# Distributed-Learning-Networking-Group/torchgpipe

Measured on AMD Instinct MI355X. Metric: U-Net(5,64) GPipe training throughput (samples/sec), higher is better.
Workload: dtype fp32; 1 GPU; model=U-Net(5,64), experiment=pipeline-1, global_batch=80, input=3x192x192, chunks=2, checkpoint=except_last, parallelism=pp1, transport=none, fused_cells=True, cell_streams=0, overlap_recompute=True, overlap_forward=True, graph_cells=False, hw_queues=4

## Files before the change

torchgpipe_amd/csrc/bindings.cpp:

```cpp
#include <algorithm>
#include <torch/extension.h>
#include <ATen/hip/HIPContext.h>
#include <ATen/hip/impl/HIPGuardImplMasqueradingAsCUDA.h>

#include <vector>

#include "aten_checks.h"
#include "kernels.h"

namespace tgpipe {
namespace {

hipStream_t stream_of(const at::Tensor& t) {
  return at::hip::getCurrentHIPStream(t.device().index()).stream();
}

const int64_t* rng_state(const c10::optional<at::Tensor>& rng, const at::Device& device) {
  if (!rng.has_value() || !rng->defined()) return nullptr;
  TORCH_CHECK(rng->is_cuda() && rng->device() == device && rng->scalar_type() == at::kLong &&
                  rng->is_contiguous() && rng->numel() == 2,
              "rng must be a contiguous int64 [2] (seed, offset) tensor on the op's device");
  return rng->data_ptr<int64_t>();
}

// ... 232 lines not shown
              "input too large for the F(4x4) kernel (needs < 1 GiB); use wino_conv");
  const float* bptr = nullptr;
  if (bias.has_value() && bias->defined()) {
    check_f32_gpu(*bias, "bias");
    TORCH_CHECK(bias->numel() == out_channels, "bias must have K elements");
    bptr = bias->data_ptr<float>();
  }
  c10::hip::HIPGuardMasqueradingAsCUDA guard(x.device());
  auto y = at::empty({n, out_channels, h, w}, x.options());
  if (y.numel() == 0) return y;
  TORCH_CHECK(variant == -1 || wino4_variant_known(static_cast<int>(variant)),
              "variant must be -1, 4-10, 12, 14-18, 20-22 or 24");
  const WinoPlan plan = wino4_plan(n, r, h, w, out_channels, static_cast<int>(variant),
                                   static_cast<int>(splits));
  at::Tensor ws;
  if (plan.workspace > 0) ws = at::empty({plan.workspace}, x.options());
  launch_wino4_conv(x.data_ptr<float>(), u.data_ptr<float>(), bptr, y.data_ptr<float>(),
                    plan.workspace > 0 ? ws.data_ptr<float>() : nullptr, n, r, h, w,
                    out_channels, plan, stream_of(x));
  return y;
}

at::Tensor wgrad_destination(const c10::optional<at::Tensor>& into, const at::Tensor& x,
                             int64_t k, int64_t c) {
  if (!into.has_value()) return at::empty({k, c, 3, 3}, x.options());
  const at::Tensor& d = *into;
  TORCH_CHECK(d.is_contiguous() && d.scalar_type() == at::kFloat && d.device() == x.device() &&
                  d.dim() == 4 && d.size(0) == k && d.size(1) == c && d.size(2) == 3 &&
                  d.size(3) == 3,
              "into must be a contiguous fp32 [K][C][3][3] tensor on x's device");
  return d;
}

at::Tensor wino_wgrad(const at::Tensor& x_in, const at::Tensor& dy_in, int64_t splits,
                      int64_t variant, const c10::optional<at::Tensor>& into) {
  auto x = x_in.contiguous();
  auto dy = dy_in.contiguous();
  check_f32_gpu(x, "x");
  check_f32_gpu(dy, "dy");
  TORCH_CHECK(x.dim() == 4 && dy.dim() == 4, "x and dy must be NCHW");
  const int64_t n = x.size(0), c = x.size(1), h = x.size(2), w = x.size(3), k = dy.size(1);
  TORCH_CHECK(dy.size(0) == n && dy.size(2) == h && dy.size(3) == w,
              "dy must be [N][K][H][W] of a 3x3/s1/p1 convolution of x");
  TORCH_CHECK(dy.device() == x.device(), "x and dy must share a device");
  TORCH_CHECK(c * h * w < (int64_t{1} << 31) && k * h * w < (int64_t{1} << 31),
              "plane too large for 32-bit channel offsets");
  c10::hip::HIPGuardMasqueradingAsCUDA guard(x.device());
  const bool accum = into.has_value();
  auto dw = wgrad_destination(into, x, k, c);
  if (n == 0 || h == 0 || w == 0) return accum ? dw : dw.zero_();
  TORCH_CHECK(variant == -1 || variant == 0 || variant == 2, "variant must be -1, 0 or 2");
  const int64_t tiles = n * ((h + 1) / 2) * ((w + 1) / 2);
  int v = variant >= 0 ? static_cast<int>(variant) : (k <= 32 ? 0 : 2);
  if (v == 2 && tiles >= (int64_t{1} << 24)) v = 0;
  const int64_t steps = (tiles + 7) / 8;
  const int s = static_cast<int>(std::min<int64_t>(
      splits > 0 ? splits : wino_wgrad_splits(n, c, k, h, w, v), steps));
  at::Tensor ws;
  if (s > 1) ws = at::empty({s * k * c * 9}, x.options());
  launch_wino_wgrad(x.data_ptr<float>(), dy.data_ptr<float>(), dw.data_ptr<float>(),
                    s > 1 ? ws.data_ptr<float>() : nullptr, n, c, k, h, w, s, v, accum,
                    stream_of(x));
  return dw;
}

at::Tensor wino4_wgrad(const at::Tensor& x_in, const at::Tensor& dy_in, int64_t splits,
                       int64_t variant, const c10::optional<at::Tensor>& into) {
  auto x = x_in.contiguous();
  auto dy = dy_in.contiguous();
  check_f32_gpu(x, "x");
  check_f32_gpu(dy, "dy");
  TORCH_CHECK(x.dim() == 4 && dy.dim() == 4, "x and dy must be NCHW");
  const int64_t n = x.size(0), c = x.size(1), h = x.size(2), w = x.size(3), k = dy.size(1);
  TORCH_CHECK(dy.size(0) == n && dy.size(2) == h && dy.size(3) == w,
              "dy must be [N][K][H][W] of a 3x3/s1/p1 convolution of x");
  TORCH_CHECK(dy.device() == x.device(), "x and dy must share a device");
  c10::hip::HIPGuardMasqueradingAsCUDA guard(x.device());
  const bool accum = into.has_value();
  auto dw = wgrad_destination(into, x, k, c);
  if (n == 0 || h == 0 || w == 0 || c == 0 || k == 0) return accum ? dw : dw.zero_();
  TORCH_CHECK(wino4_wgrad_supported(n, c, k, h, w),
              "input too large for the F(4x4) weight-gradient kernel (needs < 1 GiB); "
              "use wino_wgrad");
  TORCH_CHECK(variant >= 0 && variant <= 3,
              "variant must be 0 (fused), 1 (non-fused), 2 (split-bf16 batched GEMM) or 3 (fused, "
              "x rows through LDS)");
  const WinoPlan plan = wino4_wgrad_plan(n, c, k, h, w, static_cast<int>(variant),
                                         static_cast<int>(splits));
  at::Tensor ws;
  if (plan.workspace > 0) ws = at::empty({plan.workspace}, x.options());
  launch_wino4_wgrad(x.data_ptr<float>(), dy.data_ptr<float>(), dw.data_ptr<float>(),
                     plan.workspace > 0 ? ws.data_ptr<float>() : nullptr, n, c, k, h, w, plan,
                     accum, stream_of(x));
  return dw;
}

at::Tensor bg_weight(const at::Tensor& w, bool flip, int64_t kind,
                     const c10::optional<at::Tensor>& out, int64_t emu) {
  check_f32_gpu(w, "weight");
  TORCH_CHECK(w.dim() == 4 && w.size(2) == 3 && w.size(3) == 3, "weight must be [K][C][3][3]");
  auto wc = w.contiguous();
  const int64_t out_channels = flip ? w.size(1) : w.size(0);
  const int64_t red_channels = flip ? w.size(0) : w.size(1);
  c10::hip::HIPGuardMasqueradingAsCUDA guard(w.device());
  TORCH_CHECK(kind == 4 || kind == 2, "kind must be 4 (F(4x4)) or 2 (F(2x2))");
  auto a =
      transform_out(out, {bg_weight_numel(out_channels, red_channels, static_cast<int>(kind),
                                          static_cast<int>(emu))}, w);
  launch_bg_weight(wc.data_ptr<float>(), a.data_ptr<float>(), out_channels, red_channels, flip,
                   static_cast<int>(kind), stream_of(w), static_cast<int>(emu));
  return a;
}

at::Tensor bg_conv(const at::Tensor& x_in, const at::Tensor& a,
                   const c10::optional<at::Tensor>& bias, int64_t out_channels, int64_t bn,
                   int64_t splits, int64_t kind, int64_t waves, int64_t sub, int64_t emu,
                   const c10::optional<at::Tensor>& stats) {
  auto x = x_in.contiguous();
  check_f32_gpu(x, "x");
  check_f32_gpu(a, "a");
  TORCH_CHECK(x.dim() == 4, "x must be NCHW");
  const int64_t n = x.size(0), r = x.size(1), h = x.size(2), w = x.size(3);
  TORCH_CHECK(kind == 4 || kind == 2, "kind must be 4 (F(4x4)) or 2 (F(2x2))");
  TORCH_CHECK(a.dim() == 1 && a.numel() == bg_weight_numel(out_channels, r, static_cast<int>(kind),
                                                           static_cast<int>(emu)),
              "batched-GEMM transformed weight does not match the input/output channels");
  TORCH_CHECK(a.device() == x.device(), "a must live on the input's device");
  TORCH_CHECK(wino4_supported(n, r, h, w, out_channels),
              "input too large for the F(4x4) kernels (needs < 1 GiB)");
  const float* bptr = nullptr;
  if (bias.has_value() && bias->defined()) {
    check_f32_gpu(*bias, "bias");
    TORCH_CHECK(bias->numel() == out_channels, "bias must have K elements");
    bptr = bias->data_ptr<float>();
  }
  c10::hip::HIPGuardMasqueradingAsCUDA guard(x.device());
  auto y = at::empty({n, out_channels, h, w}, x.options());
  if (n == 0 || h == 0 || w == 0 || out_channels == 0) return y;
  const BgPlan plan = bg_plan(n, r, h, w, out_channels, static_cast<int>(bn),
                              static_cast<int>(splits), static_cast<int>(kind),
                              static_cast<int>(waves), static_cast<int>(sub),
                              static_cast<int>(emu));
  TORCH_CHECK(plan.ksteps * 16 * plan.np < (int64_t{1} << 31) &&
                  plan.mp * plan.np < (int64_t{1} << 31),
              "operands too large for the batched-GEMM kernels");
  float* pm = nullptr;
  int ipg = 0;
  if (stats.has_value() && stats->defined()) {
    check_f32_gpu(*stats, "stats");
    ipg = bg_stats_ipg(n, h, w, static_cast<int>(kind));
    const int64_t groups = (n + ipg - 1) / ipg;
    TORCH_CHECK(stats->device() == x.device() && stats->is_contiguous() &&
                    stats->numel() == 2 * groups * out_channels,
                "stats must be a contiguous [2][ceil(n / bg_stats_ipg)][K] float32 tensor");
    pm = stats->data_ptr<float>();
  }
  auto ws = at::empty({plan.workspace}, x.options());
  launch_bg_conv(x.data_ptr<float>(), a.data_ptr<float>(), bptr, y.data_ptr<float>(),
                 ws.data_ptr<float>(), n, r, h, w, out_channels, plan, stream_of(x), pm,
                 pm == nullptr ? nullptr : pm + stats->numel() / 2, ipg);
  return y;
}

int64_t bg_stats_images(int64_t n, int64_t h, int64_t w, int64_t kind) {
  return bg_stats_ipg(n, h, w, static_cast<int>(kind));
}

int64_t wino4_splits(int64_t n, int64_t c, int64_t k, int64_t h, int64_t w, int64_t variant) {
  if (variant == 0) return wino4_wgrad_plan(n, c, k, h, w, 0, 0).splits;
// ... 88 lines not shown
```

torchgpipe_amd/csrc/winograd_f4.hip:

```cpp
#include <hip/hip_runtime.h>
#include <stdint.h>

#include <algorithm>
#include <cstdlib>
#include <string>
#include <type_traits>

#include "kernels.h"

namespace tgpipe {
namespace {

typedef float floatx4 __attribute__((ext_vector_type(4)));
typedef float floatx2 __attribute__((ext_vector_type(2)));

constexpr int kP = 36;
constexpr int kC = 4;
constexpr int kOPad = 64;
constexpr int kT = 32;
constexpr int kVImg = kC * kT * kP;

template <int OG>
struct F4Cfg {
  static constexpr int kO = 16 * OG;
// ... 1979 lines not shown
  char* const vmine =
      vimg + (pt >> 4) * kEBlock + (((pc >> 3) * 16 + (pt & 15)) * 8 + (pc & 7)) * 2;
  const uint32_t chunk_bytes = static_cast<uint32_t>(kEC) * HW * 4;

  const int g = lane >> 4, row = lane & 15;
  const int a32 = wo * kEBlock + ((g & 1) * 16 + row) * 16;
  const int a16 = wo * kEBlock + 512 + ((g >> 1) * 16 + row) * 16 + (g & 1) * 8;
  const int b32 = wt * kEBlock + lane * 16;
  const int b16 = wt * kEBlock + ((g >> 1) * 16 + row) * 16 + (g & 1) * 8;

  const char* const ubase = reinterpret_cast<const char*>(u);
  const int64_t ochunk = static_cast<int64_t>(Op / 64);
  auto issue_slice = [&](int chunk, int pg, int slot) {
    const char* src = ubase + ((static_cast<int64_t>(chunk) * ochunk + ob) * kP + pg * kEPG) * 4 *
                                  kEBlock;
    char* dst = uring + slot * kEUSlice;
#pragma unroll
    for (int i = 0; i < 3; ++i) {
      const int piece = i * 8 + wave;
      __builtin_amdgcn_global_load_lds((glob_void_t*)(src + piece * 1024 + lane * 16),
                                       (lds_void_t*)(dst + piece * 1024), 16, 0, 0);
    }
  };

  if (c_begin < c_end) issue_slice(c_begin, 0, 0);
  for (int ck = c_begin; ck < c_end; ++ck) {
    f4_load_patch<kVec>(p, xr, ck * chunk_bytes);
    if (ck * kEC + pc >= R) {
#pragma unroll
      for (int b = 0; b < kP; ++b) p.d[b] = 0.f;
    }
    f4_transform(p);
#pragma unroll
    for (int b = 0; b < kP; ++b) {
      const __bf16 h = static_cast<__bf16>(p.d[b]);
      const __bf16 m = static_cast<__bf16>(p.d[b] - static_cast<float>(h));
      *reinterpret_cast<__bf16*>(vmine + b * 2 * kEBlock) = h;
      *reinterpret_cast<__bf16*>(vmine + b * 2 * kEBlock + 512) = m;
    }
    __syncthreads();
#pragma unroll
    for (int pg = 0; pg < kP / kEPG; ++pg) {
      const int slot = pg & 1;
      if (pg + 1 < kP / kEPG) {
        issue_slice(ck, pg + 1, slot ^ 1);
      } else if (ck + 1 < c_end) {
        issue_slice(ck + 1, 0, slot ^ 1);
      }
      const char* us = uring + slot * kEUSlice;
#pragma unroll
      for (int hq = 0; hq < kEPG; hq += 3) {
        bf16x8 fa[3], fb[3];
        shortx4 ga[3], gb[3];
#pragma unroll
        for (int q = 0; q < 3; ++q) {
          const int pos = pg * kEPG + hq + q;
          fa[q] = *reinterpret_cast<const bf16x8*>(us + (hq + q) * 4 * kEBlock + a32);
          fb[q] = *reinterpret_cast<const bf16x8*>(vimg + pos * 2 * kEBlock + b32);
          ga[q] = *reinterpret_cast<const shortx4*>(us + (hq + q) * 4 * kEBlock + a16);
          gb[q] = *reinterpret_cast<const shortx4*>(vimg + pos * 2 * kEBlock + b16);
        }
#pragma unroll
        for (int q = 0; q < 3; ++q) {
          const int pos = pg * kEPG + hq + q;
          acc[pos] = __builtin_amdgcn_mfma_f32_16x16x32_bf16(fa[q], fb[q], acc[pos], 0, 0, 0);
        }
#pragma unroll
        for (int q = 0; q < 3; ++q) {
          const int pos = pg * kEPG + hq + q;
          acc[pos] = __builtin_amdgcn_mfma_f32_16x16x16bf16_1k(ga[q], gb[q], acc[pos], 0, 0, 0);
        }
      }
      __builtin_amdgcn_sched_barrier(0);
      __syncthreads();
      __builtin_amdgcn_sched_barrier(0);
    }
  }

  const int tp = t0 + wt * 16 + (lane & 15);
  if (tp >= P) return;
  float* ydst = y + static_cast<int64_t>(z) * (P / tpi) * O * HW;
  f4_output_transform(acc, ydst, bias != nullptr && splits == 1 ? bias : nullptr, tp, tpi, TW,
                      H, W, O, o0 + wo * 16 + 4 * (lane >> 4));
}

__global__ __launch_bounds__(256) void bg_output_f4_kernel(
    const float* __restrict__ cbuf, const float* __restrict__ bias, float* __restrict__ y, int O,
    int Mp, int Np, int P, int tpi, int TW, int H, int W, int splits) {
  const int64_t idx = static_cast<int64_t>(blockIdx.x) * blockDim.x + threadIdx.x;
  if (idx >= static_cast<int64_t>(O) * P) return;
  const int t = static_cast<int>(idx % P);
  const int o = static_cast<int>(idx / P);
  const int64_t pos = static_cast<int64_t>(Mp) * Np;
  const float* src = cbuf + static_cast<int64_t>(o) * Np + t;
  float m[kP];
#pragma unroll
  for (int b = 0; b < kP; ++b) m[b] = src[b * pos];
  for (int z = 1; z < splits; ++z) {
    const float* sz = src + static_cast<int64_t>(z) * kP * pos;
#pragma unroll
    for (int b = 0; b < kP; ++b) m[b] += sz[b * pos];
  }
  float s[4][6];
#pragma unroll
  for (int jc = 0; jc < 6; ++jc) {
    const float a = m[6 + jc] + m[12 + jc], bq = m[6 + jc] - m[12 + jc];
    const float cc = m[18 + jc] + m[24 + jc], d = m[18 + jc] - m[24 + jc];
    s[0][jc] = m[jc] + a + cc;
    s[1][jc] = bq + 2.f * d;
    s[2][jc] = a + 4.f * cc;
    s[3][jc] = bq + 8.f * d + m[30 + jc];
  }
  const float bv = bias ? bias[o] : 0.f;
  const int n = t / tpi;
  const int rem = t - n * tpi;
  const int ty = rem / TW;
  const int py = 4 * ty, px = 4 * (rem - ty * TW);
  float* yp = y + (static_cast<int64_t>(n) * O + o) * H * W + static_cast<int64_t>(py) * W + px;
  const bool full = (W & 3) == 0 && py + 4 <= H;
#pragma unroll
  for (int k = 0; k < 4; ++k) {
    const float a = s[k][1] + s[k][2], bq = s[k][1] - s[k][2];
    const float cc = s[k][3] + s[k][4], d = s[k][3] - s[k][4];
    const floatx4 out{s[k][0] + a + cc + bv, bq + 2.f * d + bv, a + 4.f * cc + bv,
                      bq + 8.f * d + s[k][5] + bv};
    if (full) {
      *reinterpret_cast<floatx4*>(yp + k * W) = out;
    } else if (py + k < H) {
#pragma unroll
      for (int l = 0; l < 4; ++l)
        if (px + l < W) yp[k * W + l] = out[l];
    }
  }
}

constexpr int kP2 = 16;

__device__ __forceinline__ void f2_weight_tile(const float* __restrict__ w, int O, int R, int m,
                                               int r, bool flip, float (&v)[kP2]) {
  float g[3][3] = {};
  if (r < R && m < O) {
    const float* src = flip ? w + (static_cast<int64_t>(r) * O + m) * 9
                            : w + (static_cast<int64_t>(m) * R + r) * 9;
#pragma unroll
    for (int i = 0; i < 3; ++i)
#pragma unroll
      for (int jc = 0; jc < 3; ++jc) g[i][jc] = flip ? src[(2 - i) * 3 + (2 - jc)] : src[i * 3 + jc];
  }
  float t[4][3];
#pragma unroll
  for (int jc = 0; jc < 3; ++jc) {
    t[0][jc] = g[0][jc];
    t[1][jc] = 0.5f * (g[0][jc] + g[1][jc] + g[2][jc]);
    t[2][jc] = 0.5f * (g[0][jc] - g[1][jc] + g[2][jc]);
    t[3][jc] = g[2][jc];
  }
#pragma unroll
  for (int i = 0; i < 4; ++i) {
    v[i * 4 + 0] = t[i][0];
    v[i * 4 + 1] = 0.5f * (t[i][0] + t[i][1] + t[i][2]);
    v[i * 4 + 2] = 0.5f * (t[i][0] - t[i][1] + t[i][2]);
    v[i * 4 + 3] = t[i][2];
  }
}


// ... 752 lines not shown
  hipLaunchKernelGGL(plan.kind == 2 ? bg_output_f2_kernel : bg_output_f4_kernel,
                     dim3(static_cast<unsigned>((ot + 255) / 256)), dim3(256),
                     0, stream, cbuf, bias, y, static_cast<int>(out_channels),
                     static_cast<int>(plan.mp), static_cast<int>(plan.np), static_cast<int>(P),
                     static_cast<int>(th * tw), static_cast<int>(tw), static_cast<int>(h),
                     static_cast<int>(w), plan.splits);
}



namespace {
struct WgEmuPlan {
  int64_t ksteps, mp, np;
  int bn;
};

WgEmuPlan wg_emu_plan(int64_t n, int64_t c, int64_t k, int64_t h, int64_t w) {
  WgEmuPlan p;
  const int64_t P = n * ((h + 3) / 4) * ((w + 3) / 4);
  p.ksteps = (P + 15) / 16;
  p.bn = bg_pick_bn(c, 4, true);
  p.mp = bg_round(k, 128);
  p.np = bg_round(c, p.bn);
  return p;
}

int wg_emu_splits(const WgEmuPlan& p) {
  const int64_t tiles = (p.mp / 128) * (p.np / p.bn) * kP;
  int64_t s = 1;
  while (tiles * s < 1024 && p.ksteps / (s * 2) >= 8) s *= 2;
  return static_cast<int>(s);
}

int64_t wg_emu_workspace(const WgEmuPlan& p, int splits) {
  return bg_image_numel(kP, p.ksteps, p.mp + p.np, true) +
         static_cast<int64_t>(splits) * kP * p.mp * p.np;
}

void launch_wgrad_emu(const float* x, const float* dy, float* dw, float* ws, int64_t n,
                      int64_t c, int64_t k, int64_t h, int64_t w, int splits, bool accum,
                      hipStream_t stream) {
  const WgEmuPlan p = wg_emu_plan(n, c, k, h, w);
  const int64_t th = (h + 3) / 4, tw = (w + 3) / 4;
  const int64_t P = n * th * tw;
  float* am = ws;
  float* bv = am + bg_image_numel(kP, p.ksteps, p.mp, true);
  float* cb = bv + bg_image_numel(kP, p.ksteps, p.np, true);
  const bool vec = (w & 3) == 0;
  const int64_t mt = p.ksteps * 4 * p.mp, vt = p.ksteps * 4 * p.np;
  hipLaunchKernelGGL(vec ? wg_dy_emu_kernel<true> : wg_dy_emu_kernel<false>,
                     dim3(static_cast<unsigned>((mt + 255) / 256)), dim3(256), 0, stream, dy, am,
                     static_cast<int>(n), static_cast<int>(k), static_cast<int>(h),
                     static_cast<int>(w), static_cast<int>(th), static_cast<int>(tw),
                     static_cast<int>(p.mp), static_cast<int>(p.ksteps),
                     static_cast<uint32_t>(n * k * h * w * 4));
  hipLaunchKernelGGL(vec ? wg_x_emu_kernel<true> : wg_x_emu_kernel<false>,
                     dim3(static_cast<unsigned>((vt + 255) / 256)), dim3(256), 0, stream, x, bv,
                     static_cast<int>(c), static_cast<int>(h), static_cast<int>(w),
                     static_cast<int>(tw), static_cast<int>(th * tw), static_cast<int>(P),
                     static_cast<int>(p.np), static_cast<int>(p.ksteps),
                     static_cast<uint32_t>(n * c * h * w * 4));
  const int mtiles = static_cast<int>(p.mp / 128);
  const int ntiles = static_cast<int>(p.np / p.bn);
  const int64_t nwg = static_cast<int64_t>(mtiles) * ntiles * kP * splits;
  auto gemm = bg_emu_gemm(p.bn);
  hipLaunchKernelGGL(gemm, dim3(static_cast<unsigned>(nwg)), dim3(256), 0, stream, am, bv, cb,
                     static_cast<int>(p.mp), static_cast<int>(p.np), static_cast<int>(p.ksteps),
                     mtiles, ntiles, static_cast<int>(kP), splits);
  const int64_t ot = k * c;
  hipLaunchKernelGGL(wg_output_emu_kernel, dim3(static_cast<unsigned>((ot + 255) / 256)),
                     dim3(256), 0, stream, cb, dw, static_cast<int>(k), static_cast<int>(c),
                     static_cast<int>(p.mp), static_cast<int>(p.np), splits, accum);
}
}


bool wino4_wgrad_supported(int64_t n, int64_t c, int64_t k, int64_t h, int64_t w) {
  const int64_t lim = (int64_t{1} << 30) - 64;
  const int64_t tiles = n * ((h + 3) / 4) * ((w + 3) / 4);
  return n * c * h * w * 4 < lim && n * k * h * w * 4 < lim && n * c * h * w > 0 &&
         n * k * h * w > 0 && tiles + 64 < (int64_t{1} << 30);
}

WinoPlan wino4_wgrad_plan(int64_t n, int64_t c, int64_t k, int64_t h, int64_t w, int variant,
                          int splits) {
  WinoPlan plan;
  plan.variant = variant >= 1 && variant <= 3 ? variant : 0;
  if (plan.variant == 3 && ((w & 3) != 0 || w < 16)) plan.variant = 0;
  const int64_t tiles = n * ((h + 3) / 4) * ((w + 3) / 4);
  const int64_t cpad = (c + 31) / 32 * 32, kpad = (k + 63) / 64 * 64;
  const bool emu = plan.variant == 2;
  const WgEmuPlan p = wg_emu_plan(n, c, k, h, w);
  const int64_t steps = emu ? (tiles + 15) / 16 : (tiles + 3) / 4;
  int64_t s = splits;
  if (s <= 0 && emu) s = wg_emu_splits(p);
  if (s <= 0) {
    const double mb = static_cast<double>(cpad) * kpad * 9 * 4 / 1e6;
    s = split_k_by_cost((cpad / 32) * (kpad / 64), steps, 256, 2.5, 5.0, 0.8, mb, 512);
  }
  plan.splits = static_cast<int>(std::min(s, steps));
  plan.workspace = plan.splits > 1 ? plan.splits * k * c * 9 : 0;
  if (plan.variant == 1) plan.workspace += steps * 4 * (cpad + kpad) * kP;
  if (emu) plan.workspace = wg_emu_workspace(p, plan.splits);
  return plan;
}

void launch_wino4_wgrad(const float* x, const float* dy, float* dw, float* ws, int64_t n,
                        int64_t c, int64_t k, int64_t h, int64_t w, const WinoPlan& plan,
                        bool accum, hipStream_t stream) {
  const int splits = plan.splits;
  if (plan.variant == 2) {
    launch_wgrad_emu(x, dy, dw, ws, n, c, k, h, w, splits, accum, stream);
    return;
  }
  const int64_t th = (h + 3) / 4, tw = (w + 3) / 4;
  const int64_t P = n * th * tw;
  const int cblocks = static_cast<int>((c + 31) / 32);
  const int kblocks = static_cast<int>((k + 63) / 64);
  const int64_t nwg = static_cast<int64_t>(cblocks) * kblocks * splits;
  const uint32_t x_bytes = static_cast<uint32_t>(n * c * h * w * 4);
  const uint32_t dy_bytes = static_cast<uint32_t>(n * k * h * w * 4);
  float* partial = ws;
  if (plan.variant == 1) {
    const int64_t nsteps = (P + 3) / 4;
    const int64_t ppad = nsteps * 4;
    float* vx = ws;
    float* m = vx + ppad * cblocks * 32 * kP;
    partial = m + ppad * kblocks * 64 * kP;
    const int64_t vt = ppad * cblocks * 32, mt = ppad * kblocks * 64;
    hipLaunchKernelGGL(f4_wg_vx_kernel, dim3(static_cast<unsigned>((vt + 255) / 256)), dim3(256), 0,
                       stream, x, vx, static_cast<int>(n), static_cast<int>(c), static_cast<int>(h),
                       static_cast<int>(w), static_cast<int>(th), static_cast<int>(tw),
                       static_cast<int>(ppad), cblocks, vt, x_bytes);
    auto mk = (w & 3) == 0 ? f4_wg_mdy_kernel<true> : f4_wg_mdy_kernel<false>;
    hipLaunchKernelGGL(mk, dim3(static_cast<unsigned>((mt + 255) / 256)), dim3(256), 0, stream, dy,
                       m, static_cast<int>(n), static_cast<int>(k), static_cast<int>(h),
                       static_cast<int>(w), static_cast<int>(th), static_cast<int>(tw),
                       static_cast<int>(ppad), kblocks, mt, dy_bytes);
    hipLaunchKernelGGL(f4_wgrad_gemm_kernel<>, dim3(static_cast<unsigned>(nwg)), dim3(kWgThreads), 0,
                       stream, vx, m, splits > 1 ? partial : dw, static_cast<int>(c),
                       static_cast<int>(k), static_cast<int>(nsteps), cblocks, kblocks, splits,
                       accum && splits == 1);
  } else {
    auto kernel = (w & 3) == 0 ? f4_wgrad_kernel<true> : f4_wgrad_kernel<false>;
    if (plan.variant == 3) kernel = f4_wgrad_rows_kernel;
    hipLaunchKernelGGL(kernel, dim3(static_cast<unsigned>(nwg)), dim3(kWgThreads), 0,
                       stream, x, dy, splits > 1 ? partial : dw, static_cast<int>(n),
                       static_cast<int>(c), static_cast<int>(k), static_cast<int>(h),
                       static_cast<int>(w), static_cast<int>(th), static_cast<int>(tw),
                       static_cast<int>(P), cblocks, kblocks, splits, x_bytes, dy_bytes,
                       accum && splits == 1);
  }
  if (splits > 1) {
    launch_split_reduce(partial, nullptr, dw, k * c * 9, 9, static_cast<int>(k), splits, stream,
                        accum);
  }
}

}
```

torchgpipe_amd/ops/conv.py:

```python
import os
import threading
from typing import Any, Dict, List, Optional, Sequence, Tuple
import weakref

import torch
from torch import Tensor, nn
import torch.nn.functional as F

from torchgpipe_amd.ops import _ext, gradacc, precision
from torchgpipe_amd.ops.precision import autocast_lowp

__all__ = ['WinogradConv2d', 'winograd_conv2d', 'wino_eligible', 'new_step',
           'clear_winograd_caches', 'cache_bytes', 'refresh_step_caches', 'hold_cache',
           'size_cache_budget', 'conv_with_bn_stats']

_STEP = 0
_CACHE_BYTES: Dict[torch.device, int] = {}
_BUDGET: Optional[int] = None
_DEVICE_BUDGET: Dict[torch.device, int] = {}
_FRACTION = os.environ.get('TGPIPE_WINOGRAD_CACHE_FRACTION')
CACHE_PEAK_FRACTION: Optional[float] = float(_FRACTION) if _FRACTION else None
PRESPLIT_MB = max(0, int(os.environ.get('TGPIPE_CG_PRESPLIT_MB', '2048')))


# ... 315 lines not shown
        db = None
        if ctx.has_bias and ctx.needs_input_grad[2]:
            db = dy.sum((0, 2, 3))
        return dx, dw, db, None


class _WinogradConvStats(torch.autograd.Function):

    @staticmethod
    def forward(ctx, x: Tensor, weight: Tensor, cache: _TransformCache,
                kind: int) -> Tuple[Tensor, Tensor]:
        ops = _ext.require(x)
        x = x.contiguous()
        n, _, h, w = x.shape
        k = weight.shape[0]
        groups = -(-n // ops.bg_stats_images(n, h, w, kind))
        stats = torch.empty(2, groups, k, device=x.device, dtype=torch.float32)
        y = ops.bg_conv(x, cache.get(weight, False, bg=kind), None, k, 0, 0, kind,
                        stats=stats)
        ctx.save_for_backward(x, weight)
        ctx.cache = cache
        ctx.param = weight
        ctx.mark_non_differentiable(stats)
        ctx.set_materialize_grads(False)
        return y, stats

    @staticmethod
    def backward(ctx, dy: Optional[Tensor], _dstats: Optional[Tensor]):
        if dy is None:
            ctx.param = None
            return None, None, None, None
        x, weight = ctx.saved_tensors
        dx, dw = _conv_grads(x, weight, dy.contiguous(), ctx.cache, ctx.needs_input_grad[0],
                             ctx.needs_input_grad[1], ctx.param)
        ctx.param = None
        return dx, dw, None, None


BG_BN_STATS = os.environ.get('TGPIPE_BG_BN_STATS', '1') != '0'


def conv_with_bn_stats(module: nn.Conv2d, x: Tensor
                       ) -> Optional[Tuple[Tensor, Tensor, int]]:
    if not BG_BN_STATS or module.bias is not None:
        return None
    kind = _bg_kind(x, module.out_channels)
    if not kind:
        return None
    y, stats = _WinogradConvStats.apply(x, module.weight, module._wino, kind)
    n, _, h, w = x.shape
    return y, stats, _ext.require(x).bg_stats_images(n, h, w, kind)


def _conv_grads(x: Tensor, weight: Tensor, dy: Tensor, cache: _TransformCache, need_x: bool,
                need_w: bool, param: Optional[Tensor] = None
                ) -> Tuple[Optional[Tensor], Optional[Tensor]]:
    dx = dw = None
    if need_x:
        dx = _conv(dy, cache, weight, None, True)
    if need_w:
        ops = _ext.require(dy)
        f4, mfma = _wgrad_f4(x, dy, weight), _wgrad_on_mfma(x, weight)
        fuse, into = gradacc.target(param) if param is not None else (False, None)
        if f4:
            dw = ops.wino4_wgrad(x, dy, 0, _wgrad_f4_variant(x, weight), into)
        elif mfma:
            dw = ops.wino_wgrad(x, dy, 0, -1, into)
        else:
            dw = torch.ops.aten.convolution_backward(
                dy, x, weight, None, [1, 1], [1, 1], [1, 1], False, [0, 0], 1,
                [False, True, False])[1]
        if fuse:
            assert param is not None
            if into is None:
                gradacc.commit(param, dw)
            elif not (f4 or mfma):
                into.add_(dw)
            dw = None
    return dx, dw


WGRAD_EMU = os.environ.get('TGPIPE_WGRAD_EMU', '1') != '0'
WGRAD_EMU_MIN_TILES = 320


def _wgrad_f4_variant(x: Tensor, weight: Tensor) -> int:
    if min(weight.shape[0], weight.shape[1]) < 512:
        return 3 if x.shape[3] % 4 == 0 and x.shape[3] >= F4_ROWS_MIN_WIDTH else 0
    tiles = x.shape[0] * -(-x.shape[2] // 4) * -(-x.shape[3] // 4)
    return 2 if WGRAD_EMU and tiles >= WGRAD_EMU_MIN_TILES else 1


def _wgrad_f4(x: Tensor, dy: Tensor, weight: Tensor) -> bool:
    plane = min(x.shape[2], x.shape[3])
    wide = min(weight.shape[0], weight.shape[1]) >= F4_WIDE_CHANNELS
    return (F4_ENABLED and weight.shape[1] >= 16
            and (plane >= F4_MIN_PLANE or (plane >= F4_MIN_PLANE_WIDE and wide))
            and x.numel() * x.element_size() < F4_MAX_BYTES
            and dy.numel() * dy.element_size() < F4_MAX_BYTES)


def _wgrad_on_mfma(x: Tensor, weight: Tensor) -> bool:
    k, c = weight.shape[0], weight.shape[1]
    if k > 32:
        return c >= 16
    return c >= 64 and x.shape[2] * x.shape[3] >= 96 * 96


MIN_CHANNELS = 8


WINOGRAD_ENABLED = os.environ.get('TGPIPE_WINOGRAD', '1') != '0'

MAX_TRANSFORM_BYTES = int(float(os.environ.get('TGPIPE_WINOGRAD_MAX_TRANSFORM_MB', '2048'))
                          * (1 << 20))


WEIGHT_DOMINATED_RATIO = float(os.environ.get('TGPIPE_WINOGRAD_WEIGHT_RATIO', '256'))


def _transform_ratio(x: Tensor, weight: Tensor) -> float:
    positions = 16 if min(x.shape[2], x.shape[3]) < F4_MIN_PLANE else 36
    return weight.shape[0] * weight.shape[1] * positions / max(1, x.numel())


def wino_eligible(x: Tensor, weight: Tensor, stride: Sequence[int] = (1, 1),
                  padding: Sequence[int] = (1, 1), dilation: Sequence[int] = (1, 1),
                  groups: int = 1) -> bool:
    return (WINOGRAD_ENABLED and x.is_cuda and x.dim() == 4 and x.dtype == torch.float32
            and not autocast_lowp('cuda')
            and weight.shape[1] >= MIN_CHANNELS
            and weight.shape[0] * weight.shape[1] * 16 * 4 <= MAX_TRANSFORM_BYTES
            and weight.dtype == torch.float32 and tuple(weight.shape[2:]) == (3, 3)
            and tuple(stride) == (1, 1) and tuple(padding) == (1, 1)
            and tuple(dilation) == (1, 1) and groups == 1
            and _transform_ratio(x, weight) <= WEIGHT_DOMINATED_RATIO)


def winograd_conv2d(x: Tensor, weight: Tensor, bias: Optional[Tensor] = None,
                    cache: Optional[_TransformCache] = None) -> Tensor:
    if not wino_eligible(x, weight):
        return F.conv2d(x, weight, bias, padding=1)
    return _WinogradConv.apply(x, weight, bias, cache or _TransformCache())


class WinogradConv2d(nn.Conv2d):

    def __init__(self, *args, **kwargs) -> None:
        super().__init__(*args, **kwargs)
        self._wino = _TransformCache()

    def forward(self, input: Tensor) -> Tensor:
        if self.padding_mode == 'zeros' and wino_eligible(input, self.weight, self.stride,
                                                          self.padding, self.dilation,
                                                          self.groups):
            return _WinogradConv.apply(input, self.weight, self.bias, self._wino)
        from torchgpipe_amd.ops.convbn import gemm_conv2d, gemm_conv_eligible
        if WINOGRAD_ENABLED and self.weight.shape[1] < MIN_CHANNELS and \
                gemm_conv_eligible(input, self):
            return gemm_conv2d(input, self)
        return super().forward(input)

    def __getstate__(self):
        state = self.__dict__.copy()
        state['_wino'] = _TransformCache()
        return state
```

Before: 720.1 samples/sec.

## Add fused split-bf16 F(4x4) Winograd weight-gradient kernel for small-channel layers

Adds a new weight-gradient kernel variant (4) that transforms x and dy tiles in LDS, splits each value into three bf16 parts, and accumulates with bf16 MFMAs to emulate fp32 precision. It uses 32x32 channel blocks with two wave phases that each handle half of the 36 Winograd positions, then reduces the halves through LDS. The dispatcher routes specific (C,K,W) shape classes at width 192 to this variant. The goal is faster wgrad on the full-resolution layers, at the cost of slightly different numerics and a shape-specific heuristic.

```diff
diff --git a/torchgpipe_amd/csrc/bindings.cpp b/torchgpipe_amd/csrc/bindings.cpp
--- a/torchgpipe_amd/csrc/bindings.cpp
+++ b/torchgpipe_amd/csrc/bindings.cpp
@@ -338,9 +338,9 @@
   TORCH_CHECK(wino4_wgrad_supported(n, c, k, h, w),
               "input too large for the F(4x4) weight-gradient kernel (needs < 1 GiB); "
               "use wino_wgrad");
-  TORCH_CHECK(variant >= 0 && variant <= 3,
-              "variant must be 0 (fused), 1 (non-fused), 2 (split-bf16 batched GEMM) or 3 (fused, "
-              "x rows through LDS)");
+  TORCH_CHECK(variant >= 0 && variant <= 4,
+              "variant must be 0 (fused), 1 (non-fused), 2 (split-bf16 batched GEMM), 3 (fused, "
+              "x rows through LDS) or 4 (fused, split-bf16)");
   const WinoPlan plan = wino4_wgrad_plan(n, c, k, h, w, static_cast<int>(variant),
                                          static_cast<int>(splits));
   at::Tensor ws;
diff --git a/torchgpipe_amd/csrc/winograd_f4.hip b/torchgpipe_amd/csrc/winograd_f4.hip
--- a/torchgpipe_amd/csrc/winograd_f4.hip
+++ b/torchgpipe_amd/csrc/winograd_f4.hip
@@ -2085,6 +2085,160 @@
   float* ydst = y + static_cast<int64_t>(z) * (P / tpi) * O * HW;
   f4_output_transform(acc, ydst, bias != nullptr && splits == 1 ? bias : nullptr, tp, tpi, TW,
                       H, W, O, o0 + wo * 16 + 4 * (lane >> 4));
+}
+
+constexpr int kWeT = 8;
+constexpr int kWePlane = 64 * kWeT * 2;
+constexpr int kWePos = 3 * kWePlane + 16;
+constexpr int kWeImg = kP * kWePos;
+constexpr int kWeHalf = kP / 2;
+typedef __bf16 bf16x2 __attribute__((ext_vector_type(2)));
+
+__device__ __forceinline__ float f4_we_round(float v) {
+  return __builtin_bit_cast(float, __builtin_convertvector(floatx2{0.f, v}, bf16x2));
+}
+
+__device__ __forceinline__ void f4_we_split_store(const float (&v)[kP], char* mine) {
+#pragma unroll
+  for (int b = 0; b < kP; ++b) {
+    const float h = f4_we_round(v[b]);
+    const float r = v[b] - h;
+    const float m = f4_we_round(r);
+    const float l = f4_we_round(r - m);
+    uint16_t* dst = reinterpret_cast<uint16_t*>(mine + b * kWePos);
+    dst[0] = static_cast<uint16_t>(__float_as_uint(h) >> 16);
+    dst[kWePlane / 2] = static_cast<uint16_t>(__float_as_uint(m) >> 16);
+    dst[kWePlane] = static_cast<uint16_t>(__float_as_uint(l) >> 16);
+  }
+}
+
+__device__ __forceinline__ void f4_cursor_advance8(F4TileCursor& cur, int TH, int TW) {
+  f4_cursor_advance(cur, TH, TW);
+  f4_cursor_advance(cur, TH, TW);
+}
+
+__global__ __launch_bounds__(kWgThreads, 1) void f4_wgrad_emu_kernel(
+    const float* __restrict__ x, const float* __restrict__ dy, float* __restrict__ dw, int N,
+    int C, int K, int H, int W, int TH, int TW, int P, int cblocks, int kblocks, int splits,
+    uint32_t x_bytes, uint32_t dy_bytes, bool accum) {
+  __shared__ __attribute__((aligned(16))) char lds[kWeImg];
+
+  const int nwg = cblocks * kblocks * splits;
+  const int bid = blockIdx.x;
+  const int xcd = bid & 7;
+  const int qq = nwg >> 3, rr = nwg & 7;
+  const int wgid = (xcd < rr ? xcd * (qq + 1) : rr * (qq + 1) + (xcd - rr) * qq) + (bid >> 3);
+  const int cb = wgid % cblocks;
+  const int kb = (wgid / cblocks) % kblocks;
+  const int z = wgid / (cblocks * kblocks);
+
+  const int tid = threadIdx.x;
+  const int lane = tid & 63;
+  const int wave = __builtin_amdgcn_readfirstlane(tid >> 6);
+  const int wk = wave & 1;
+  const int wc = (wave >> 1) & 1;
+  const int ph = wave >> 2;
+  const int c0 = cb * 32;
+  const int k0 = kb * 32;
+
+  const int nsteps = (P + kWeT - 1) / kWeT;
+  const int s_begin = static_cast<int>(static_cast<int64_t>(z) * nsteps / splits);
+  const int s_end = static_cast<int>(static_cast<int64_t>(z + 1) * nsteps / splits);
+  floatx4 acc[kWeHalf];
+#pragma unroll
+  for (int i = 0; i < kWeHalf; ++i) acc[i] = floatx4{0.f, 0.f, 0.f, 0.f};
+
+  const int g = lane >> 4, row = lane & 15;
+  const char* const pbase = lds + ph * kWeHalf * kWePos;
+  const int arow = (wk * 16 + row) * 16, brow = (32 + wc * 16 + row) * 16;
+  const int a32 = (g == 2 ? 1 : 0) * kWePlane + arow;
+  const int b32 = (g == 1 ? 1 : g == 3 ? 2 : 0) * kWePlane + brow;
+  const int a16 = (g < 2 ? 2 : 1) * kWePlane + arow + (g & 1) * 8;
+  const int b16 = (g < 2 ? 0 : 1) * kWePlane + brow + (g & 1) * 8;
+
+  auto multiply = [&]() {
+#pragma unroll
+    for (int i0 = 0; i0 < kWeHalf; i0 += 3) {
+      bf16x8 fa[3], fb[3];
+      shortx4 ga[3], gb[3];
+#pragma unroll
+      for (int q = 0; q < 3; ++q) {
+        const char* pos = pbase + (i0 + q) * kWePos;
+        fa[q] = *reinterpret_cast<const bf16x8*>(pos + a32);
+        fb[q] = *reinterpret_cast<const bf16x8*>(pos + b32);
+        ga[q] = *reinterpret_cast<const shortx4*>(pos + a16);
+        gb[q] = *reinterpret_cast<const shortx4*>(pos + b16);
+      }
+#pragma unroll
+      for (int q = 0; q < 3; ++q)
+        acc[i0 + q] = __builtin_amdgcn_mfma_f32_16x16x32_bf16(fa[q], fb[q], acc[i0 + q], 0, 0, 0);
+#pragma unroll
+      for (int q = 0; q < 3; ++q)
+        acc[i0 + q] =
+            __builtin_amdgcn_mfma_f32_16x16x16bf16_1k(ga[q], gb[q], acc[i0 + q], 0, 0, 0);
+    }
+  };
+  auto barrier = [&]() {
+    __builtin_amdgcn_sched_barrier(0);
+    __syncthreads();
+    __builtin_amdgcn_sched_barrier(0);
+  };
+
+  const int t = tid & 7;
+  const int r = (tid >> 3) & 31;
+  F4TileCursor cur = f4_cursor_at(kWeT * s_begin + t, TH, TW);
+  if (wave < 4) {
+    const __amdgpu_buffer_rsrc_t xr =
+        __builtin_amdgcn_make_buffer_rsrc(const_cast<float*>(x), static_cast<short>(0),
+                                          static_cast<int>(x_bytes), 0x00020000);
+    char* const mine = lds + (32 + r) * 16 + t * 2;
+    F4Patch p;
+    f4_patch_offsets(p, cur, c0 + r, N, C, H, W);
+    f4_load_patch<true>(p, xr, 0);
+    for (int s = s_begin; s < s_end; ++s) {
+      f4_transform(p);
+      f4_we_split_store(p.d, mine);
+      f4_cursor_advance8(cur, TH, TW);
+      f4_patch_offsets(p, cur, c0 + r, N, C, H, W);
+      f4_load_patch<true>(p, xr, 0);
+      barrier();
+      multiply();
+      barrier();
+    }
+  } else {
+    const __amdgpu_buffer_rsrc_t dyr =
+        __builtin_amdgcn_make_buffer_rsrc(const_cast<float*>(dy), static_cast<short>(0),
+                                          static_cast<int>(dy_bytes), 0x00020000);
+    char* const mine = lds + r * 16 + t * 2;
+    float gt[16];
+    f4_load_dy<true>(gt, dyr, cur, k0 + r, N, K, H, W);
+    for (int s = s_begin; s < s_end; ++s) {
+      float m[kP];
+      f4_dy_transform(gt, m);
+      f4_we_split_store(m, mine);
+      f4_cursor_advance8(cur, TH, TW);
+      f4_load_dy<true>(gt, dyr, cur, k0 + r, N, K, H, W);
+      barrier();
+      multiply();
+      barrier();
+    }
+  }
+
+  floatx4* const xch = reinterpret_cast<floatx4*>(lds);
+  if (ph == 1) {
+#pragma unroll
+    for (int i = 0; i < kWeHalf; ++i) xch[((wave & 3) * kWeHalf + i) * 64 + lane] = acc[i];
+  }
+  __syncthreads();
+  if (ph == 1) return;
+  floatx4 full[kP];
+#pragma unroll
+  for (int i = 0; i < kWeHalf; ++i) {
+    full[i] = acc[i];
+    full[kWeHalf + i] = xch[(wave * kWeHalf + i) * 64 + lane];
+  }
+  f4_wgrad_epilogue(full, dw + static_cast<int64_t>(z) * K * C * 9, c0 + wc * 16 + (lane & 15),
+                    k0 + wk * 16 + 4 * (lane >> 4), C, K, accum);
 }
 
 __global__ __launch_bounds__(256) void bg_output_f4_kernel(
@@ -3003,11 +3157,13 @@
          n * k * h * w > 0 && tiles + 64 < (int64_t{1} << 30);
 }
 
+constexpr double kWgEmuStepUs = 4.0;
+
 WinoPlan wino4_wgrad_plan(int64_t n, int64_t c, int64_t k, int64_t h, int64_t w, int variant,
                           int splits) {
   WinoPlan plan;
-  plan.variant = variant >= 1 && variant <= 3 ? variant : 0;
-  if (plan.variant == 3 && ((w & 3) != 0 || w < 16)) plan.variant = 0;
+  plan.variant = variant >= 1 && variant <= 4 ? variant : 0;
+  if (plan.variant >= 3 && ((w & 3) != 0 || w < 16)) plan.variant = 0;
   const int64_t tiles = n * ((h + 3) / 4) * ((w + 3) / 4);
   const int64_t cpad = (c + 31) / 32 * 32, kpad = (k + 63) / 64 * 64;
   const bool emu = plan.variant == 2;
@@ -3015,6 +3171,17 @@
   const int64_t steps = emu ? (tiles + 15) / 16 : (tiles + 3) / 4;
   int64_t s = splits;
   if (s <= 0 && emu) s = wg_emu_splits(p);
+  if (plan.variant == 4) {
+    const int64_t chunks = (tiles + kWeT - 1) / kWeT;
+    if (s <= 0) {
+      const double mb = static_cast<double>(cpad) * ((k + 31) / 32 * 32) * 9 * 4 / 1e6;
+      s = split_k_by_cost((cpad / 32) * ((k + 31) / 32), chunks, 256, kWgEmuStepUs, 5.0, 0.8, mb,
+                          512);
+    }
+    plan.splits = static_cast<int>(std::min(s, chunks));
+    plan.workspace = plan.splits > 1 ? plan.splits * k * c * 9 : 0;
+    return plan;
+  }
   if (s <= 0) {
     const double mb = static_cast<double>(cpad) * kpad * 9 * 4 / 1e6;
     s = split_k_by_cost((cpad / 32) * (kpad / 64), steps, 256, 2.5, 5.0, 0.8, mb, 512);
@@ -3037,7 +3204,7 @@
   const int64_t th = (h + 3) / 4, tw = (w + 3) / 4;
   const int64_t P = n * th * tw;
   const int cblocks = static_cast<int>((c + 31) / 32);
-  const int kblocks = static_cast<int>((k + 63) / 64);
+  const int kblocks = static_cast<int>(plan.variant == 4 ? (k + 31) / 32 : (k + 63) / 64);
   const int64_t nwg = static_cast<int64_t>(cblocks) * kblocks * splits;
   const uint32_t x_bytes = static_cast<uint32_t>(n * c * h * w * 4);
   const uint32_t dy_bytes = static_cast<uint32_t>(n * k * h * w * 4);
@@ -3065,6 +3232,7 @@
   } else {
     auto kernel = (w & 3) == 0 ? f4_wgrad_kernel<true> : f4_wgrad_kernel<false>;
     if (plan.variant == 3) kernel = f4_wgrad_rows_kernel;
+    if (plan.variant == 4) kernel = f4_wgrad_emu_kernel;
     hipLaunchKernelGGL(kernel, dim3(static_cast<unsigned>(nwg)), dim3(kWgThreads), 0,
                        stream, x, dy, splits > 1 ? partial : dw, static_cast<int>(n),
                        static_cast<int>(c), static_cast<int>(k), static_cast<int>(h),
diff --git a/torchgpipe_amd/ops/conv.py b/torchgpipe_amd/ops/conv.py
--- a/torchgpipe_amd/ops/conv.py
+++ b/torchgpipe_amd/ops/conv.py
@@ -421,11 +421,16 @@
 
 WGRAD_EMU = os.environ.get('TGPIPE_WGRAD_EMU', '1') != '0'
 WGRAD_EMU_MIN_TILES = 320
+WGRAD_FUSED_EMU_CLASSES = frozenset({(128, 32, 192), (32, 32, 192)})
 
 
 def _wgrad_f4_variant(x: Tensor, weight: Tensor) -> int:
     if min(weight.shape[0], weight.shape[1]) < 512:
-        return 3 if x.shape[3] % 4 == 0 and x.shape[3] >= F4_ROWS_MIN_WIDTH else 0
+        rows = x.shape[3] % 4 == 0 and x.shape[3] >= F4_ROWS_MIN_WIDTH
+        if (rows and WGRAD_EMU
+                and (weight.shape[1], weight.shape[0], x.shape[3]) in WGRAD_FUSED_EMU_CLASSES):
+            return 4
+        return 3 if rows else 0
     tiles = x.shape[0] * -(-x.shape[2] // 4) * -(-x.shape[3] // 4)
     return 2 if WGRAD_EMU and tiles >= WGRAD_EMU_MIN_TILES else 1
 
```

After: 719.3 samples/sec. No clear change (-0.1%).
